# armlabstanford/Touch-GS

Hardware: AMD Instinct MI355X
Metric: train iters/s (whole-job views/s) + render Mpix/s, 1M Gaussians @ 1080p (higher is better)
Workload: dtype f32; 1 GPU; configs[2]: 1M Gaussians, 1080p, full Touch-GS train loop (RGB L1/SSIM + tactile depth/uncertainty loss), one view per rank per iter; gaussians=1000000, width=1920, height=1080, sh_degree=3, views=8, tiles=8160, longest_tile_list_any_view=792, max_list_hint=1022, parallelism=dp1, layout=morton (model.spatial_sort(): same scene, rows permuted), depth_loss_type=DEPTH_UNCERTAINTY_WEIGHTED_LOSS

## Files before the change

### touch_gs_amd/csrc/imgloss.hip

```cpp
#include <math.h>
#include <stdlib.h>
#include "tgs_common.h"

namespace {

constexpr int WIN = 11, HALO = 5;
struct Win { float g[WIN]; };
#ifdef TGS_SSIM_SGPR_WINDOW
#define WK(k) win.g[k]
#else
__device__ constexpr float WGT[WIN] = {0x1.0d956cp-10f, 0x1.f1fe02p-8f, 0x1.26eb18p-5f, 0x1.bff0fep-4f, 0x1.b43c4p-3f,
                                       0x1.10656p-2f, 0x1.b43c4p-3f, 0x1.bff0fep-4f, 0x1.26eb18p-5f, 0x1.f1fe02p-8f,
                                       0x1.0d956cp-10f};
#define WK(k) WGT[k]
#endif

#ifndef TGS_SSIM_DMA
#define TGS_SSIM_DMA 0
#endif
constexpr int SW = 64;
constexpr int NTH = 3 * SW;
constexpr int RB = WIN;
__host__ __device__ constexpr int seg_rows(int nblk) { return RB * nblk - 2 * HALO; }

template <int CH>
struct RowBlock {
  static constexpr int ROWF = (SW + 2 * HALO) * CH;
  static constexpr int NIT = (RB * ROWF + NTH - 1) / NTH;
  template <int B = 8>
  static __device__ __forceinline__ void stage(const float* __restrict__ src, float* __restrict__ lds,
                                               int W, int H, int x0, int r0, int tid) {
#pragma unroll 1
    for (int it0 = 0; it0 < NIT; it0 += B) {
      float v[B];
#pragma unroll
      for (int u = 0; u < B; u++) {
        const int i = tid + NTH * (it0 + u);
        const int j = i / ROWF, e = i - j * ROWF;
        const int gy = r0 + j, gxf = (x0 - HALO) * CH + e;
        v[u] = 0.f;
        if (i < RB * ROWF && gy >= 0 && gy < H && gxf >= 0 && gxf < W * CH) v[u] = src[(size_t)gy * W * CH + gxf];
      }
#pragma unroll
      for (int u = 0; u < B; u++) {
        const int i = tid + NTH * (it0 + u);
        if (i < RB * ROWF) lds[i] = v[u];
      }
    }
  }
  static constexpr int PADF = (RB * ROWF + TGS_WAVE - 1) / TGS_WAVE * TGS_WAVE;
  static constexpr int NDMA = PADF / TGS_WAVE;
  static __device__ __forceinline__ void dma(__amdgpu_buffer_rsrc_t rsrc, float* __restrict__ lds, int W, int H, int x0, int r0, int tid) {
    typedef __attribute__((address_space(3))) float lds_float;
    const int wave = __builtin_amdgcn_readfirstlane(tid >> 6), lane = tid & 63;
    constexpr int NW = NTH / TGS_WAVE;
    const int gx0 = (x0 - HALO) * CH, WC = W * CH;
#pragma unroll
    for (int u = 0; u * NW < NDMA; u++) {
      const int chunk = u * NW + wave;
      if (chunk < NDMA) {
        const int i = chunk * TGS_WAVE + lane;
        const int j = i / ROWF, e = i - j * ROWF;
        const int gy = r0 + j, gxf = gx0 + e;
        const bool in = i < RB * ROWF && (unsigned)gy < (unsigned)H && (unsigned)gxf < (unsigned)WC;
        const unsigned off = in ? (unsigned)(gy * WC + gxf) * 4u : 0xffffffffu;
        __builtin_amdgcn_raw_ptr_buffer_load_lds(rsrc, (lds_float*)(lds + chunk * TGS_WAVE), 4, off, 0, 0, 0);
      }
    }
  }
  static __device__ __forceinline__ void stage2(const float* __restrict__ src_a, const float* __restrict__ src_b,
                                                float* __restrict__ lds_a, float* __restrict__ lds_b,
                                                int W, int H, int x0, int r0, int tid) {
#ifndef TGS_SSIM_FWD_B
#define TGS_SSIM_FWD_B 13
#endif
    constexpr int B = TGS_SSIM_FWD_B;
#pragma unroll 1
    for (int it0 = 0; it0 < NIT; it0 += B) {
      float va[B], vb[B];
#pragma unroll
      for (int u = 0; u < B; u++) {
        const int i = tid + NTH * (it0 + u);
        const int j = i / ROWF, e = i - j * ROWF;
        const int gy = r0 + j, gxf = (x0 - HALO) * CH + e;
        va[u] = 0.f; vb[u] = 0.f;
        if (it0 + u < NIT && i < RB * ROWF && gy >= 0 && gy < H && gxf >= 0 && gxf < W * CH) {
          const size_t o = (size_t)gy * W * CH + gxf;
          va[u] = src_a[o]; vb[u] = src_b[o];
        }
      }
#pragma unroll
      for (int u = 0; u < B; u++) {
        const int i = tid + NTH * (it0 + u);
        if (it0 + u < NIT && i < RB * ROWF) { lds_a[i] = va[u]; lds_b[i] = vb[u]; }
      }
    }
  }
};

__global__ __launch_bounds__(NTH) __attribute__((amdgpu_waves_per_eu(4, 8))) void k_ssim_fwd(int W, int H, Win win,
                                                  const float* __restrict__ img,
                                                  const float* __restrict__ gt,
                                                  float* __restrict__ adj ,
                                                  float* __restrict__ block_partials, int n_partials, int NBLK,
                                                  int y_lo, int y_hi, int c_lo, int c_hi) {
  const int SEG = seg_rows(NBLK);
  constexpr int ROWF = RowBlock<3>::ROWF;
#if TGS_SSIM_DMA & 1
  __shared__ float sa2[2][RowBlock<3>::PADF], sb2[2][RowBlock<3>::PADF];
  const __amdgpu_buffer_rsrc_t rs_a = __builtin_amdgcn_make_buffer_rsrc((void*)img, 0, (int)((size_t)W * H * 12), 0x00020000);
  const __amdgpu_buffer_rsrc_t rs_b = __builtin_amdgcn_make_buffer_rsrc((void*)gt, 0, (int)((size_t)W * H * 12), 0x00020000);
#else
  __shared__ float sa[RB * ROWF], sb[RB * ROWF];
#endif
  __shared__ float red[NTH / TGS_WAVE];
  const int tid = threadIdx.x;
  const int x0 = blockIdx.x * SW, ys = y_lo + blockIdx.y * SEG;
  const int gx = x0 + tid / 3, c = tid - (tid / 3) * 3;
  const int ye = min(ys + SEG, y_hi);
  float w[RB][5];
#pragma unroll
  for (int p = 0; p < RB; p++)
#pragma unroll
    for (int q = 0; q < 5; q++) w[p][q] = 0.f;
  float msum = 0.f;
#if TGS_SSIM_DMA & 1
  RowBlock<3>::dma(rs_a, sa2[0], W, H, x0, ys - HALO, tid);
  RowBlock<3>::dma(rs_b, sb2[0], W, H, x0, ys - HALO, tid);
#endif
  for (int blk = 0; blk < NBLK; blk++) {
    const int r0 = ys - HALO + blk * RB;
    if (r0 - HALO >= ye) break;
#if TGS_SSIM_DMA & 1
    asm volatile("s_waitcnt vmcnt(0)" ::: "memory");
    __syncthreads();
    if (blk + 1 < NBLK && r0 + RB - HALO < ye) {
      RowBlock<3>::dma(rs_a, sa2[(blk + 1) & 1], W, H, x0, r0 + RB, tid);
      RowBlock<3>::dma(rs_b, sb2[(blk + 1) & 1], W, H, x0, r0 + RB, tid);
    }
    const float* sa = sa2[blk & 1];
    const float* sb = sb2[blk & 1];
#else
    __syncthreads();
    {
      RowBlock<3>::stage2(img, gt, sa, sb, W, H, x0, r0, tid);
    }
    __syncthreads();
#endif
#pragma unroll
    for (int p = 0; p < RB; p++) {
      const float* ra = sa + p * ROWF + tid;
      const float* rb = sb + p * ROWF + tid;
      float m1 = 0.f, m2 = 0.f, e11 = 0.f, e22 = 0.f, e12 = 0.f;
#pragma unroll
      for (int k = 0; k < WIN; k++) {
        const float a = ra[3 * k], b = rb[3 * k];
        const float ga = WK(k) * a, gb = WK(k) * b;
        m1 += ga; m2 += gb;
        e11 = fmaf(ga, a, e11); e22 = fmaf(gb, b, e22); e12 = fmaf(ga, b, e12);
      }
      w[p][0] = m1; w[p][1] = m2; w[p][2] = e11; w[p][3] = e22; w[p][4] = e12;
      const int gy = r0 + p - HALO;
      if (gy >= ys && gy < ye) {
        float o[5] = {0.f, 0.f, 0.f, 0.f, 0.f};
#pragma unroll
        for (int k = 0; k < WIN; k++) {
#pragma unroll
          for (int q = 0; q < 5; q++) o[q] = fmaf(WK(k), w[(p + 1 + k) % RB][q], o[q]);
        }
        const float C1 = 0.01f * 0.01f, C2 = 0.03f * 0.03f;
        const float mu1 = o[0], mu2 = o[1];
        const float s11 = o[2] - mu1 * mu1, s22 = o[3] - mu2 * mu2, s12 = o[4] - mu1 * mu2;
        const float n1 = 2.f * mu1 * mu2 + C1, n2 = 2.f * s12 + C2;
        const float d1 = mu1 * mu1 + mu2 * mu2 + C1, d2 = s11 + s22 + C2;
        const float id1 = __builtin_amdgcn_rcpf(d1), id2 = __builtin_amdgcn_rcpf(d2);
        const float m = n1 * n2 * id1 * id2;
        if (gx < W) {
          if (gy >= c_lo && gy < c_hi) msum += m;
          if (adj) {
            const float dm_ds12 = 2.f * n1 * id1 * id2;
            const float dm_ds11 = -m * id2;
            const float dm_dmu1 = 2.f * mu2 * n2 * id1 * id2 - m * 2.f * mu1 * id1;
            float* o3 = adj + (((size_t)gy * W + gx) * 3 + c) * 3;
            o3[0] = dm_dmu1 - 2.f * mu1 * dm_ds11 - mu2 * dm_ds12;
            o3[1] = dm_ds11;
            o3[2] = dm_ds12;
          }
        }
      }
    }
  }
  const float tot = wave_sum(msum);
  if ((tid & 63) == 0) red[tid >> 6] = tot;
  __syncthreads();
  const int wg = blockIdx.y * gridDim.x + blockIdx.x, nwg = gridDim.x * gridDim.y;
  if (tid == 0) block_partials[wg] = red[0] + red[1] + red[2];
  for (int i = nwg + wg * NTH + tid; i < n_partials; i += nwg * NTH) block_partials[i] = 0.f;
}

__global__ __launch_bounds__(NTH) __attribute__((amdgpu_waves_per_eu(4, 8))) void k_ssim_bwd(int W, int H, Win win, float weight,
                                                  const float* __restrict__ img,
                                                  const float* __restrict__ gt,
                                                  const float* __restrict__ adj,
                                                  float* __restrict__ v_img, int NBLK, int y_lo, int y_hi) {
  const int SEG = seg_rows(NBLK);
  constexpr int ROWF = RowBlock<9>::ROWF;
#if TGS_SSIM_DMA & 2
  __shared__ float sadj2[2][RowBlock<9>::PADF];
  const __amdgpu_buffer_rsrc_t rs_j = __builtin_amdgcn_make_buffer_rsrc((void*)adj, 0, (int)((size_t)W * H * 36), 0x00020000);
#else
  __shared__ float sadj[RB * ROWF];
#endif
  const int tid = threadIdx.x;
  const int x0 = blockIdx.x * SW, ys = y_lo + blockIdx.y * SEG;
  const int gx = x0 + tid / 3;
  const int ye = min(ys + SEG, y_hi);
  float w[RB][3];
#pragma unroll
  for (int p = 0; p < RB; p++) { w[p][0] = 0.f; w[p][1] = 0.f; w[p][2] = 0.f; }
#if TGS_SSIM_DMA & 2
  RowBlock<9>::dma(rs_j, sadj2[0], W, H, x0, ys - HALO, tid);
#endif
  for (int blk = 0; blk < NBLK; blk++) {
    const int r0 = ys - HALO + blk * RB;
    if (r0 - HALO >= ye) break;
#if TGS_SSIM_DMA & 2
    asm volatile("s_waitcnt vmcnt(0)" ::: "memory");
    __syncthreads();
    if (blk + 1 < NBLK && r0 + RB - HALO < ye) RowBlock<9>::dma(rs_j, sadj2[(blk + 1) & 1], W, H, x0, r0 + RB, tid);
    const float* sadj = sadj2[blk & 1];
#else
    __syncthreads();
    {
#ifndef TGS_SSIM_BWD_B
#define TGS_SSIM_BWD_B 20
#endif
      RowBlock<9>::stage<TGS_SSIM_BWD_B>(adj, sadj, W, H, x0, r0, tid);
    }
    __syncthreads();
#endif
#pragma unroll
    for (int p = 0; p < RB; p++) {
      const float* r = sadj + p * ROWF + 3 * tid;
      float h0 = 0.f, h1 = 0.f, h2 = 0.f;
#pragma unroll
      for (int k = 0; k < WIN; k++) {
        h0 = fmaf(WK(k), r[9 * k], h0);
        h1 = fmaf(WK(k), r[9 * k + 1], h1);
        h2 = fmaf(WK(k), r[9 * k + 2], h2);
      }
      w[p][0] = h0; w[p][1] = h1; w[p][2] = h2;
      const int gy = r0 + p - HALO;
      if (gy >= ys && gy < ye) {
        float o0 = 0.f, o1 = 0.f, o2 = 0.f;
#pragma unroll
        for (int k = 0; k < WIN; k++) {
          o0 = fmaf(WK(k), w[(p + 1 + k) % RB][0], o0);
          o1 = fmaf(WK(k), w[(p + 1 + k) % RB][1], o1);
          o2 = fmaf(WK(k), w[(p + 1 + k) % RB][2], o2);
        }
        if (gx < W) {
          const size_t pidx = (size_t)gy * W * 3 + (size_t)x0 * 3 + tid;
          v_img[pidx] = weight * (o0 + 2.f * img[pidx] * o1 + gt[pidx] * o2);
        }
      }
    }
  }
}


constexpr int SWO = SW - 2 * HALO;
__host__ __device__ constexpr int fused_seg_rows(int nblk) { return RB * nblk - 4 * HALO; }

__global__ __launch_bounds__(NTH) __attribute__((amdgpu_waves_per_eu(3, 4))) void k_ssim_fused(
    int W, int H, float weight, const float* __restrict__ img, const float* __restrict__ gt,
    float* __restrict__ v_img, float* __restrict__ block_partials, int n_partials, int NBLK,
    int y_lo, int y_hi, int c_lo, int c_hi) {
  const int SEG = fused_seg_rows(NBLK);
  constexpr int ROWF = RowBlock<3>::ROWF;
  constexpr int ADJF = SW * 9;
  __shared__ float sa[RB * ROWF], sb[RB * ROWF];
  __shared__ float sadj[RB * ADJF];
  __shared__ float red[NTH / TGS_WAVE];
  const int tid = threadIdx.x;
  const int col = tid / 3, c = tid - col * 3;
  const int xa0 = blockIdx.x * SWO - HALO;
  const int gx = xa0 + col;
  const int ys = y_lo + blockIdx.y * SEG, ye = min(ys + SEG, y_hi);
  const bool own_col = col >= HALO && col < SW - HALO;
  const int cb = min(max(col - HALO, 0), SWO - 1);
  float w[RB][5], w2[RB][3];
#pragma unroll
  for (int p = 0; p < RB; p++) {
#pragma unroll
    for (int q = 0; q < 5; q++) w[p][q] = 0.f;
    w2[p][0] = 0.f; w2[p][1] = 0.f; w2[p][2] = 0.f;
  }
  float msum = 0.f;
  for (int blk = 0; blk < NBLK; blk++) {
    const int r0 = ys - 2 * HALO + blk * RB;
    if (r0 - 2 * HALO >= ye) break;
    __syncthreads();
    RowBlock<3>::stage2(img, gt, sa, sb, W, H, xa0, r0, tid);
    __syncthreads();
#pragma unroll
    for (int p = 0; p < RB; p++) {
      const float* ra = sa + p * ROWF + tid;
      const float* rb = sb + p * ROWF + tid;
      float m1 = 0.f, m2 = 0.f, e11 = 0.f, e22 = 0.f, e12 = 0.f;
#pragma unroll
      for (int k = 0; k < WIN; k++) {
        const float a = ra[3 * k], b = rb[3 * k];
        const float ga = WK(k) * a, gb = WK(k) * b;
        m1 += ga; m2 += gb;
        e11 = fmaf(ga, a, e11); e22 = fmaf(gb, b, e22); e12 = fmaf(ga, b, e12);
      }
      w[p][0] = m1; w[p][1] = m2; w[p][2] = e11; w[p][3] = e22; w[p][4] = e12;
      const int gy = r0 + p - HALO;
      float A = 0.f, B = 0.f, C = 0.f;
      if (gy >= ys - HALO && gy < ye + HALO && gy >= 0 && gy < H) {
        float o[5] = {0.f, 0.f, 0.f, 0.f, 0.f};
#pragma unroll
        for (int k = 0; k < WIN; k++) {
#pragma unroll
          for (int q = 0; q < 5; q++) o[q] = fmaf(WK(k), w[(p + 1 + k) % RB][q], o[q]);
        }
        const float C1 = 0.01f * 0.01f, C2 = 0.03f * 0.03f;
        const float mu1 = o[0], mu2 = o[1];
        const float s11 = o[2] - mu1 * mu1, s22 = o[3] - mu2 * mu2, s12 = o[4] - mu1 * mu2;
        const float n1 = 2.f * mu1 * mu2 + C1, n2 = 2.f * s12 + C2;
        const float d1 = mu1 * mu1 + mu2 * mu2 + C1, d2 = s11 + s22 + C2;
        const float id1 = __builtin_amdgcn_rcpf(d1), id2 = __builtin_amdgcn_rcpf(d2);
        const float m = n1 * n2 * id1 * id2;
        if (gx >= 0 && gx < W) {
          if (own_col && gy >= ys && gy < ye && gy >= c_lo && gy < c_hi) msum += m;
          const float dm_ds12 = 2.f * n1 * id1 * id2;
          const float dm_ds11 = -m * id2;
          const float dm_dmu1 = 2.f * mu2 * n2 * id1 * id2 - m * 2.f * mu1 * id1;
          A = dm_dmu1 - 2.f * mu1 * dm_ds11 - mu2 * dm_ds12;
          B = dm_ds11;
          C = dm_ds12;
        }
      }
      float* o3 = sadj + p * ADJF + tid * 3;
      o3[0] = A; o3[1] = B; o3[2] = C;
    }
    __syncthreads();
#pragma unroll
    for (int p = 0; p < RB; p++) {
      const float* r = sadj + p * ADJF + (cb * 3 + c) * 3;
      float h0 = 0.f, h1 = 0.f, h2 = 0.f;
#pragma unroll
      for (int k = 0; k < WIN; k++) {
        h0 = fmaf(WK(k), r[9 * k], h0);
        h1 = fmaf(WK(k), r[9 * k + 1], h1);
        h2 = fmaf(WK(k), r[9 * k + 2], h2);
      }
      w2[p][0] = h0; w2[p][1] = h1; w2[p][2] = h2;
      const int gy = r0 + p - 2 * HALO;
      if (gy >= ys && gy < ye) {
        float o0 = 0.f, o1 = 0.f, o2 = 0.f;
#pragma unroll
        for (int k = 0; k < WIN; k++) {
          o0 = fmaf(WK(k), w2[(p + 1 + k) % RB][0], o0);
          o1 = fmaf(WK(k), w2[(p + 1 + k) % RB][1], o1);
          o2 = fmaf(WK(k), w2[(p + 1 + k) % RB][2], o2);
        }
        if (own_col && gx < W) {
          const size_t pidx = ((size_t)gy * W + gx) * 3 + c;
          v_img[pidx] = weight * (o0 + 2.f * img[pidx] * o1 + gt[pidx] * o2);
        }
      }
    }
  }
  const float tot = wave_sum(msum);
  if ((tid & 63) == 0) red[tid >> 6] = tot;
  __syncthreads();
  const int wg = blockIdx.y * gridDim.x + blockIdx.x, nwg = gridDim.x * gridDim.y;
  if (tid == 0) block_partials[wg] = red[0] + red[1] + red[2];
  for (int i = nwg + wg * NTH + tid; i < n_partials; i += nwg * NTH) block_partials[i] = 0.f;
}

}

static inline bool count_inside(int y0, int y1, int c0, int c1) { return c0 >= c1 || (c0 >= y0 && c1 <= y1); }

static int ssim_impl(int W, int H, const float* img, const float* gt, float weight,
                     float* block_partials, int n_partials, float* v_img, float* scratch,
                     int y0, int y1, int c0, int c1, void* stream) {
  TGS_CHECK_ARG(W > 0 && H > 0, "bad image size");
  TGS_CHECK_ARG(img && gt && block_partials, "null pointer");
  TGS_CHECK_ARG(!v_img || scratch, "gradient needs scratch");
  TGS_CHECK_ARG(0 <= y0 && y0 <= y1 && y1 <= H && y0 <= c0 && c0 <= c1 && c1 <= y1, "bad row range");
  Win win;
  double g[WIN], sum = 0.0;
  for (int i = 0; i < WIN; i++) { g[i] = exp(-(double)((i - HALO) * (i - HALO)) / (2.0 * 1.5 * 1.5)); sum += g[i]; }
  for (int i = 0; i < WIN; i++) win.g[i] = (float)(g[i] / sum);
  static const int env_nblk = [] { const char* e = getenv("TGS_SSIM_NBLK"); return e ? max(2, min(16, atoi(e))) : 0; }();
  static const int env_fused = [] { const char* e = getenv("TGS_SSIM_FUSED"); return e ? atoi(e) : 0; }();
  if (v_img && env_fused && y1 > y0 && count_inside(y0, y1, c0, c1)) {
    const int fx = (W + SWO - 1) / SWO;
    auto wgs = [&](int nb) { return (long long)fx * ((y1 - y0 + fused_seg_rows(nb) - 1) / fused_seg_rows(nb)); };
    int nblk = 7;
    while (nblk > 3 && wgs(nblk) < 600) nblk--;
    if (env_nblk) nblk = max(3, env_nblk);
    while (nblk < 16 && wgs(nblk) > n_partials) nblk++;
    TGS_CHECK_ARG(wgs(nblk) <= n_partials, "block_partials too small");
    const int SEGF = fused_seg_rows(nblk);
    hipLaunchKernelGGL(k_ssim_fused, dim3(fx, (y1 - y0 + SEGF - 1) / SEGF, 1), dim3(NTH), 0, (hipStream_t)stream, W, H, weight,
                       img, gt, v_img, block_partials, n_partials, nblk, y0, y1, c0, c1);
    TGS_CHECK_LAUNCH();
    return TGS_OK;
  }
  const int f0 = v_img ? max(0, y0 - HALO) : y0, f1 = v_img ? min(H, y1 + HALO) : y1;
  const int rows = f1 - f0;
  if (rows <= 0) return TGS_OK;
  const int sx = (W + SW - 1) / SW;
  int nblk = 4;
  while (nblk > 2 && (long long)sx * ((rows + seg_rows(nblk) - 1) / seg_rows(nblk)) < 3 * 256) nblk--;
  if (env_nblk) nblk = env_nblk;
  while (nblk < 16 && (long long)sx * ((rows + seg_rows(nblk) - 1) / seg_rows(nblk)) > n_partials) nblk++;
  TGS_CHECK_ARG((long long)sx * ((rows + seg_rows(nblk) - 1) / seg_rows(nblk)) <= n_partials, "block_partials too small");
  const int SEG = seg_rows(nblk);
  const dim3 block(NTH);
  hipStream_t s = (hipStream_t)stream;
  hipLaunchKernelGGL(k_ssim_fwd, dim3(sx, (rows + SEG - 1) / SEG, 1), block, 0, s, W, H, win, img, gt,
                     v_img ? scratch : nullptr, block_partials, n_partials, nblk, f0, f1, c0, c1);
  TGS_CHECK_LAUNCH();
  if (v_img && y1 > y0) {
    hipLaunchKernelGGL(k_ssim_bwd, dim3(sx, (y1 - y0 + SEG - 1) / SEG, 1), block, 0, s, W, H, win, weight, img, gt,
                       scratch, v_img, nblk, y0, y1);
    TGS_CHECK_LAUNCH();
  }
  return TGS_OK;
}

extern "C" int tgs_ssim_fwd_bwd(int W, int H, const float* img, const float* gt, float weight,
                                float* block_partials, float* v_img, float* scratch,
                                void* stream) {
  return ssim_impl(W, H, img, gt, weight, block_partials, ((W + 15) / 16) * ((H + 15) / 16), v_img, scratch,
                   0, H, 0, H, stream);
}

extern "C" int tgs_ssim_fwd_bwd_rows(int W, int H, const float* img, const float* gt, float weight,
                                     float* block_partials, int n_partials, float* v_img,
                                     float* scratch, int y0, int y1, int count_y0, int count_y1,
                                     void* stream) {
  return ssim_impl(W, H, img, gt, weight, block_partials, n_partials, v_img, scratch, y0, y1, count_y0,
                   count_y1, stream);
}
```

Before: 993.4 iters/s.

## Vectorize SSIM tile staging with aligned float4 loads and padded LDS rows

Replaces the scalar per-element global-to-LDS staging in the SSIM forward, backward and fused kernels with float4 loads into 4-aligned, padded LDS rows, using a per-block shift to handle misalignment. The unused buffer-load-to-LDS DMA path is removed. An optional prefetch of the next adjoint row block, plus early loads of img/gt in the backward kernel, is added behind a compile flag that is off by default. The vector path is enabled by default when the width is a multiple of 4 and pointers are 16-byte aligned. It adds edge clamping, more LDS per row and more template variants.

Result: no change. 1003 iters/s, median of 6 (+1.0%).

```diff
diff --git a/touch_gs_amd/csrc/imgloss.hip b/touch_gs_amd/csrc/imgloss.hip
--- a/touch_gs_amd/csrc/imgloss.hip
+++ b/touch_gs_amd/csrc/imgloss.hip
@@ -1,4 +1,5 @@
 #include <math.h>
+#include <stdint.h>
 #include <stdlib.h>
 #include "tgs_common.h"
 
@@ -15,8 +16,8 @@
 #define WK(k) WGT[k]
 #endif
 
-#ifndef TGS_SSIM_DMA
-#define TGS_SSIM_DMA 0
+#ifndef TGS_SSIM_PREFETCH
+#define TGS_SSIM_PREFETCH 0
 #endif
 constexpr int SW = 64;
 constexpr int NTH = 3 * SW;
@@ -26,10 +27,40 @@
 template <int CH>
 struct RowBlock {
   static constexpr int ROWF = (SW + 2 * HALO) * CH;
+  static constexpr int ROWV = (ROWF + 3 + 3) / 4 * 4;
+  static constexpr int LPR = ROWV / 4 <= TGS_WAVE ? TGS_WAVE : NTH;
+  static constexpr int RP = NTH / LPR;
+  static constexpr int NLD = (RB + RP - 1) / RP;
   static constexpr int NIT = (RB * ROWF + NTH - 1) / NTH;
+  static __device__ __forceinline__ int shift(int x0) { return ((x0 - HALO) * CH) & 3; }
+  static __device__ __forceinline__ void load(const float* __restrict__ src, float4 (&v)[NLD], int W, int H, int x0, int r0, int tid) {
+    const int sub = RP > 1 ? __builtin_amdgcn_readfirstlane(tid / LPR) : 0, c4 = RP > 1 ? tid % LPR : tid;
+    const int WC = W * CH;
+    const unsigned gxf = (unsigned)min(max((x0 - HALO) * CH - shift(x0) + 4 * c4, 0), WC - 4);
+#pragma unroll
+    for (int u = 0; u < NLD; u++) {
+      const int gy = min(max(r0 + u * RP + sub, 0), H - 1);
+      v[u] = *reinterpret_cast<const float4*>(src + (size_t)gy * WC + gxf);
+    }
+  }
+  static __device__ __forceinline__ void store(float* __restrict__ lds, const float4 (&v)[NLD], int W, int H, int x0, int r0, int tid) {
+    const int sub = RP > 1 ? __builtin_amdgcn_readfirstlane(tid / LPR) : 0, c4 = RP > 1 ? tid % LPR : tid;
+    const int sh = shift(x0);
+    const int gxf = (x0 - HALO) * CH - sh + 4 * c4;
+    const bool col_in = (unsigned)gxf < (unsigned)(W * CH);
+    if (4 * c4 < sh + ROWF) {
+#pragma unroll
+      for (int u = 0; u < NLD; u++) {
+        const int j = u * RP + sub;
+        const bool in = (unsigned)(r0 + j) < (unsigned)H && col_in;
+        if (j < RB) *reinterpret_cast<float4*>(lds + j * ROWV + 4 * c4) = in ? v[u] : make_float4(0.f, 0.f, 0.f, 0.f);
+      }
+    }
+  }
   template <int B = 8>
   static __device__ __forceinline__ void stage(const float* __restrict__ src, float* __restrict__ lds,
                                                int W, int H, int x0, int r0, int tid) {
+    const int sh = shift(x0);
 #pragma unroll 1
     for (int it0 = 0; it0 < NIT; it0 += B) {
       float v[B];
@@ -44,35 +75,17 @@
 #pragma unroll
       for (int u = 0; u < B; u++) {
         const int i = tid + NTH * (it0 + u);
-        if (i < RB * ROWF) lds[i] = v[u];
-      }
-    }
-  }
-  static constexpr int PADF = (RB * ROWF + TGS_WAVE - 1) / TGS_WAVE * TGS_WAVE;
-  static constexpr int NDMA = PADF / TGS_WAVE;
-  static __device__ __forceinline__ void dma(__amdgpu_buffer_rsrc_t rsrc, float* __restrict__ lds, int W, int H, int x0, int r0, int tid) {
-    typedef __attribute__((address_space(3))) float lds_float;
-    const int wave = __builtin_amdgcn_readfirstlane(tid >> 6), lane = tid & 63;
-    constexpr int NW = NTH / TGS_WAVE;
-    const int gx0 = (x0 - HALO) * CH, WC = W * CH;
-#pragma unroll
-    for (int u = 0; u * NW < NDMA; u++) {
-      const int chunk = u * NW + wave;
-      if (chunk < NDMA) {
-        const int i = chunk * TGS_WAVE + lane;
         const int j = i / ROWF, e = i - j * ROWF;
-        const int gy = r0 + j, gxf = gx0 + e;
-        const bool in = i < RB * ROWF && (unsigned)gy < (unsigned)H && (unsigned)gxf < (unsigned)WC;
-        const unsigned off = in ? (unsigned)(gy * WC + gxf) * 4u : 0xffffffffu;
-        __builtin_amdgcn_raw_ptr_buffer_load_lds(rsrc, (lds_float*)(lds + chunk * TGS_WAVE), 4, off, 0, 0, 0);
+        if (i < RB * ROWF) lds[j * ROWV + sh + e] = v[u];
       }
     }
   }
   static __device__ __forceinline__ void stage2(const float* __restrict__ src_a, const float* __restrict__ src_b,
                                                 float* __restrict__ lds_a, float* __restrict__ lds_b,
                                                 int W, int H, int x0, int r0, int tid) {
+    const int sh = shift(x0);
 #ifndef TGS_SSIM_FWD_B
-#define TGS_SSIM_FWD_B 13
+#define TGS_SSIM_FWD_B 7
 #endif
     constexpr int B = TGS_SSIM_FWD_B;
 #pragma unroll 1
@@ -92,12 +105,14 @@
 #pragma unroll
       for (int u = 0; u < B; u++) {
         const int i = tid + NTH * (it0 + u);
-        if (it0 + u < NIT && i < RB * ROWF) { lds_a[i] = va[u]; lds_b[i] = vb[u]; }
+        const int j = i / ROWF, e = i - j * ROWF;
+        if (it0 + u < NIT && i < RB * ROWF) { lds_a[j * ROWV + sh + e] = va[u]; lds_b[j * ROWV + sh + e] = vb[u]; }
       }
     }
   }
 };
 
+template <bool VEC>
 __global__ __launch_bounds__(NTH) __attribute__((amdgpu_waves_per_eu(4, 8))) void k_ssim_fwd(int W, int H, Win win,
                                                   const float* __restrict__ img,
                                                   const float* __restrict__ gt,
@@ -105,14 +120,9 @@
                                                   float* __restrict__ block_partials, int n_partials, int NBLK,
                                                   int y_lo, int y_hi, int c_lo, int c_hi) {
   const int SEG = seg_rows(NBLK);
-  constexpr int ROWF = RowBlock<3>::ROWF;
-#if TGS_SSIM_DMA & 1
-  __shared__ float sa2[2][RowBlock<3>::PADF], sb2[2][RowBlock<3>::PADF];
-  const __amdgpu_buffer_rsrc_t rs_a = __builtin_amdgcn_make_buffer_rsrc((void*)img, 0, (int)((size_t)W * H * 12), 0x00020000);
-  const __amdgpu_buffer_rsrc_t rs_b = __builtin_amdgcn_make_buffer_rsrc((void*)gt, 0, (int)((size_t)W * H * 12), 0x00020000);
-#else
-  __shared__ float sa[RB * ROWF], sb[RB * ROWF];
-#endif
+  typedef RowBlock<3> RBK;
+  constexpr int ROWV = RBK::ROWV;
+  __shared__ __attribute__((aligned(16))) float sa[RB * ROWV], sb[RB * ROWV];
   __shared__ float red[NTH / TGS_WAVE];
   const int tid = threadIdx.x;
   const int x0 = blockIdx.x * SW, ys = y_lo + blockIdx.y * SEG;
@@ -124,33 +134,25 @@
 #pragma unroll
     for (int q = 0; q < 5; q++) w[p][q] = 0.f;
   float msum = 0.f;
-#if TGS_SSIM_DMA & 1
-  RowBlock<3>::dma(rs_a, sa2[0], W, H, x0, ys - HALO, tid);
-  RowBlock<3>::dma(rs_b, sb2[0], W, H, x0, ys - HALO, tid);
-#endif
+  const int sh = RBK::shift(x0);
   for (int blk = 0; blk < NBLK; blk++) {
     const int r0 = ys - HALO + blk * RB;
     if (r0 - HALO >= ye) break;
-#if TGS_SSIM_DMA & 1
-    asm volatile("s_waitcnt vmcnt(0)" ::: "memory");
-    __syncthreads();
-    if (blk + 1 < NBLK && r0 + RB - HALO < ye) {
-      RowBlock<3>::dma(rs_a, sa2[(blk + 1) & 1], W, H, x0, r0 + RB, tid);
-      RowBlock<3>::dma(rs_b, sb2[(blk + 1) & 1], W, H, x0, r0 + RB, tid);
-    }
-    const float* sa = sa2[blk & 1];
-    const float* sb = sb2[blk & 1];
-#else
-    __syncthreads();
-    {
-      RowBlock<3>::stage2(img, gt, sa, sb, W, H, x0, r0, tid);
-    }
-    __syncthreads();
-#endif
+    __syncthreads();
+    if (VEC) {
+      float4 pa[RBK::NLD], pb[RBK::NLD];
+      RBK::load(img, pa, W, H, x0, r0, tid);
+      RBK::load(gt, pb, W, H, x0, r0, tid);
+      RBK::store(sa, pa, W, H, x0, r0, tid);
+      RBK::store(sb, pb, W, H, x0, r0, tid);
+    } else {
+      RBK::stage2(img, gt, sa, sb, W, H, x0, r0, tid);
+    }
+    __syncthreads();
 #pragma unroll
     for (int p = 0; p < RB; p++) {
-      const float* ra = sa + p * ROWF + tid;
-      const float* rb = sb + p * ROWF + tid;
+      const float* ra = sa + p * ROWV + sh + tid;
+      const float* rb = sb + p * ROWV + sh + tid;
       float m1 = 0.f, m2 = 0.f, e11 = 0.f, e22 = 0.f, e12 = 0.f;
 #pragma unroll
       for (int k = 0; k < WIN; k++) {
@@ -198,19 +200,16 @@
   for (int i = nwg + wg * NTH + tid; i < n_partials; i += nwg * NTH) block_partials[i] = 0.f;
 }
 
+template <bool VEC, int PF>
 __global__ __launch_bounds__(NTH) __attribute__((amdgpu_waves_per_eu(4, 8))) void k_ssim_bwd(int W, int H, Win win, float weight,
                                                   const float* __restrict__ img,
                                                   const float* __restrict__ gt,
                                                   const float* __restrict__ adj,
                                                   float* __restrict__ v_img, int NBLK, int y_lo, int y_hi) {
   const int SEG = seg_rows(NBLK);
-  constexpr int ROWF = RowBlock<9>::ROWF;
-#if TGS_SSIM_DMA & 2
-  __shared__ float sadj2[2][RowBlock<9>::PADF];
-  const __amdgpu_buffer_rsrc_t rs_j = __builtin_amdgcn_make_buffer_rsrc((void*)adj, 0, (int)((size_t)W * H * 36), 0x00020000);
-#else
-  __shared__ float sadj[RB * ROWF];
-#endif
+  typedef RowBlock<9> RBK;
+  constexpr int ROWV = RBK::ROWV;
+  __shared__ __attribute__((aligned(16))) float sadj[RB * ROWV];
   const int tid = threadIdx.x;
   const int x0 = blockIdx.x * SW, ys = y_lo + blockIdx.y * SEG;
   const int gx = x0 + tid / 3;
@@ -218,30 +217,34 @@
   float w[RB][3];
 #pragma unroll
   for (int p = 0; p < RB; p++) { w[p][0] = 0.f; w[p][1] = 0.f; w[p][2] = 0.f; }
-#if TGS_SSIM_DMA & 2
-  RowBlock<9>::dma(rs_j, sadj2[0], W, H, x0, ys - HALO, tid);
-#endif
+  const int sh = RBK::shift(x0);
+  float4 pj[RBK::NLD];
+  if (PF & 1) RBK::load(adj, pj, W, H, x0, ys - HALO, tid);
   for (int blk = 0; blk < NBLK; blk++) {
     const int r0 = ys - HALO + blk * RB;
     if (r0 - HALO >= ye) break;
-#if TGS_SSIM_DMA & 2
-    asm volatile("s_waitcnt vmcnt(0)" ::: "memory");
-    __syncthreads();
-    if (blk + 1 < NBLK && r0 + RB - HALO < ye) RowBlock<9>::dma(rs_j, sadj2[(blk + 1) & 1], W, H, x0, r0 + RB, tid);
-    const float* sadj = sadj2[blk & 1];
-#else
-    __syncthreads();
-    {
-#ifndef TGS_SSIM_BWD_B
-#define TGS_SSIM_BWD_B 20
-#endif
-      RowBlock<9>::stage<TGS_SSIM_BWD_B>(adj, sadj, W, H, x0, r0, tid);
-    }
-    __syncthreads();
-#endif
+    float ei[RB], eg[RB];
 #pragma unroll
     for (int p = 0; p < RB; p++) {
-      const float* r = sadj + p * ROWF + 3 * tid;
+      const int gy = r0 + p - HALO;
+      ei[p] = 0.f; eg[p] = 0.f;
+      if ((PF & 2) && gy >= ys && gy < ye && gx < W) {
+        const size_t pidx = (size_t)gy * W * 3 + (size_t)x0 * 3 + tid;
+        ei[p] = img[pidx]; eg[p] = gt[pidx];
+      }
+    }
+    __syncthreads();
+    if (VEC) {
+      if (!(PF & 1)) RBK::load(adj, pj, W, H, x0, r0, tid);
+      RBK::store(sadj, pj, W, H, x0, r0, tid);
+    } else {
+      RBK::stage<20>(adj, sadj, W, H, x0, r0, tid);
+    }
+    __syncthreads();
+    if ((PF & 1) && blk + 1 < NBLK && r0 + RB - HALO < ye) RBK::load(adj, pj, W, H, x0, r0 + RB, tid);
+#pragma unroll
+    for (int p = 0; p < RB; p++) {
+      const float* r = sadj + p * ROWV + sh + 3 * tid;
       float h0 = 0.f, h1 = 0.f, h2 = 0.f;
 #pragma unroll
       for (int k = 0; k < WIN; k++) {
@@ -261,7 +264,8 @@
         }
         if (gx < W) {
           const size_t pidx = (size_t)gy * W * 3 + (size_t)x0 * 3 + tid;
-          v_img[pidx] = weight * (o0 + 2.f * img[pidx] * o1 + gt[pidx] * o2);
+          if (!(PF & 2)) { ei[p] = img[pidx]; eg[p] = gt[pidx]; }
+          v_img[pidx] = weight * (o0 + 2.f * ei[p] * o1 + eg[p] * o2);
         }
       }
     }
@@ -272,19 +276,22 @@
 constexpr int SWO = SW - 2 * HALO;
 __host__ __device__ constexpr int fused_seg_rows(int nblk) { return RB * nblk - 4 * HALO; }
 
+template <bool VEC>
 __global__ __launch_bounds__(NTH) __attribute__((amdgpu_waves_per_eu(3, 4))) void k_ssim_fused(
     int W, int H, float weight, const float* __restrict__ img, const float* __restrict__ gt,
     float* __restrict__ v_img, float* __restrict__ block_partials, int n_partials, int NBLK,
     int y_lo, int y_hi, int c_lo, int c_hi) {
   const int SEG = fused_seg_rows(NBLK);
-  constexpr int ROWF = RowBlock<3>::ROWF;
+  typedef RowBlock<3> RBK;
+  constexpr int ROWV = RBK::ROWV;
   constexpr int ADJF = SW * 9;
-  __shared__ float sa[RB * ROWF], sb[RB * ROWF];
+  __shared__ __attribute__((aligned(16))) float sa[RB * ROWV], sb[RB * ROWV];
   __shared__ float sadj[RB * ADJF];
   __shared__ float red[NTH / TGS_WAVE];
   const int tid = threadIdx.x;
   const int col = tid / 3, c = tid - col * 3;
   const int xa0 = blockIdx.x * SWO - HALO;
+  const int sh = RBK::shift(xa0);
   const int gx = xa0 + col;
   const int ys = y_lo + blockIdx.y * SEG, ye = min(ys + SEG, y_hi);
   const bool own_col = col >= HALO && col < SW - HALO;
@@ -301,12 +308,20 @@
     const int r0 = ys - 2 * HALO + blk * RB;
     if (r0 - 2 * HALO >= ye) break;
     __syncthreads();
-    RowBlock<3>::stage2(img, gt, sa, sb, W, H, xa0, r0, tid);
+    if (VEC) {
+      float4 pa[RBK::NLD], pb[RBK::NLD];
+      RBK::load(img, pa, W, H, xa0, r0, tid);
+      RBK::load(gt, pb, W, H, xa0, r0, tid);
+      RBK::store(sa, pa, W, H, xa0, r0, tid);
+      RBK::store(sb, pb, W, H, xa0, r0, tid);
+    } else {
+      RBK::stage2(img, gt, sa, sb, W, H, xa0, r0, tid);
+    }
     __syncthreads();
 #pragma unroll
     for (int p = 0; p < RB; p++) {
-      const float* ra = sa + p * ROWF + tid;
-      const float* rb = sb + p * ROWF + tid;
+      const float* ra = sa + p * ROWV + sh + tid;
+      const float* rb = sb + p * ROWV + sh + tid;
       float m1 = 0.f, m2 = 0.f, e11 = 0.f, e22 = 0.f, e12 = 0.f;
 #pragma unroll
       for (int k = 0; k < WIN; k++) {
@@ -398,6 +413,8 @@
   for (int i = 0; i < WIN; i++) win.g[i] = (float)(g[i] / sum);
   static const int env_nblk = [] { const char* e = getenv("TGS_SSIM_NBLK"); return e ? max(2, min(16, atoi(e))) : 0; }();
   static const int env_fused = [] { const char* e = getenv("TGS_SSIM_FUSED"); return e ? atoi(e) : 0; }();
+  static const int env_vec = [] { const char* e = getenv("TGS_SSIM_VEC"); return e ? atoi(e) : 1; }();
+  const int vec = env_vec && W % 4 == 0 && (((uintptr_t)img | (uintptr_t)gt | (uintptr_t)scratch) & 15) == 0;
   if (v_img && env_fused && y1 > y0 && count_inside(y0, y1, c0, c1)) {
     const int fx = (W + SWO - 1) / SWO;
     auto wgs = [&](int nb) { return (long long)fx * ((y1 - y0 + fused_seg_rows(nb) - 1) / fused_seg_rows(nb)); };
@@ -407,8 +424,8 @@
     while (nblk < 16 && wgs(nblk) > n_partials) nblk++;
     TGS_CHECK_ARG(wgs(nblk) <= n_partials, "block_partials too small");
     const int SEGF = fused_seg_rows(nblk);
-    hipLaunchKernelGGL(k_ssim_fused, dim3(fx, (y1 - y0 + SEGF - 1) / SEGF, 1), dim3(NTH), 0, (hipStream_t)stream, W, H, weight,
-                       img, gt, v_img, block_partials, n_partials, nblk, y0, y1, c0, c1);
+    hipLaunchKernelGGL(vec ? k_ssim_fused<true> : k_ssim_fused<false>, dim3(fx, (y1 - y0 + SEGF - 1) / SEGF, 1), dim3(NTH), 0,
+                       (hipStream_t)stream, W, H, weight, img, gt, v_img, block_partials, n_partials, nblk, y0, y1, c0, c1);
     TGS_CHECK_LAUNCH();
     return TGS_OK;
   }
@@ -422,13 +439,16 @@
   while (nblk < 16 && (long long)sx * ((rows + seg_rows(nblk) - 1) / seg_rows(nblk)) > n_partials) nblk++;
   TGS_CHECK_ARG((long long)sx * ((rows + seg_rows(nblk) - 1) / seg_rows(nblk)) <= n_partials, "block_partials too small");
   const int SEG = seg_rows(nblk);
+  const bool pf = TGS_SSIM_PREFETCH && vec;
   const dim3 block(NTH);
   hipStream_t s = (hipStream_t)stream;
-  hipLaunchKernelGGL(k_ssim_fwd, dim3(sx, (rows + SEG - 1) / SEG, 1), block, 0, s, W, H, win, img, gt,
+  const auto kf = vec ? k_ssim_fwd<true> : k_ssim_fwd<false>;
+  const auto kb = pf ? k_ssim_bwd<true, TGS_SSIM_PREFETCH> : vec ? k_ssim_bwd<true, 0> : k_ssim_bwd<false, 0>;
+  hipLaunchKernelGGL(kf, dim3(sx, (rows + SEG - 1) / SEG, 1), block, 0, s, W, H, win, img, gt,
                      v_img ? scratch : nullptr, block_partials, n_partials, nblk, f0, f1, c0, c1);
   TGS_CHECK_LAUNCH();
   if (v_img && y1 > y0) {
-    hipLaunchKernelGGL(k_ssim_bwd, dim3(sx, (y1 - y0 + SEG - 1) / SEG, 1), block, 0, s, W, H, win, weight, img, gt,
+    hipLaunchKernelGGL(kb, dim3(sx, (y1 - y0 + SEG - 1) / SEG, 1), block, 0, s, W, H, win, weight, img, gt,
                        scratch, v_img, nblk, y0, y1);
     TGS_CHECK_LAUNCH();
   }
```
